# kscalelabs/kbot-joystick

Hardware: NVIDIA B200
Metric: env-steps/sec (obs + LSTM actor/critic + torque + terminations + rewards + GAE) (higher is better)
Workload: dtype f32 (tcgen05 2xFP16-split GEMMs, fp32 accumulate)

## Files before the change

### kbot-joystick_b200/csrc/kbs_net_tc.cu

```cuda
#include <math.h>
#include <cuda.h>
#include <stdlib.h>

#include "kbs_common.cuh"

namespace {

constexpr int kPanelRows = 128;
constexpr int kTileCols = 128;
constexpr int kUnitsPerTile = 32;
#ifndef KBS_STAGES
#define KBS_STAGES 6
#endif
constexpr int kStages = KBS_STAGES;
constexpr int kABlockBytes = 2 * 4 * kPanelRows * 16;
constexpr int kBBlockBytes = 2 * 4 * kTileCols * 16;
constexpr int kStageBytes = kABlockBytes + kBBlockBytes;
static_assert(kABlockBytes == kBBlockBytes, "the two producer lanes copy equal-sized blocks");
constexpr int kIssuers = 3;
constexpr int kProducers = 2;
constexpr int kEpiWarps = 8;
constexpr int kThreadsTC = 32 * (kIssuers + kProducers + kEpiWarps);
constexpr int kMaxBias = 1024;
constexpr int kSmemBytes = kStages * kStageBytes + 2 * kMaxBias * 4 + 256  + 1024 ;
// ... 566 lines not shown
      float m = out_s[lane * 41 + j] + P.joint_bias[j];
      m = m + in_arm[jj];
      const float y = in_lpf[jj];
      const float yn = y + P.lpf_alpha * (m - y);
      a.lpf[o] = rst ? 0.0f : yn;
      float act = yn;
      if (a.eps) act = yn + sd * in_eps[jj];
      const float a_eval = a.action_in ? in_ain[jj] : act;
      const float z = (a_eval - yn) / sd;
      s_z = s_z + (-0.5f * z * z - kHalfLog2Pi);
      s_log = s_log + logf(sd);
      if (a.action) a.action[o] = act;
      if (a.std) a.std[o] = sd;
      if (!a.ctrl) continue;
      const float target = a.ep.action_bias ? __fadd_rn(act, in_ab[jj]) : act;
      float tau = __fsub_rn(__fmul_rn(in_kp[jj], __fsub_rn(target, in_q[jj])), __fmul_rn(in_kd[jj], in_qd[jj]));
      if (a.ep.torque_bias) tau = __fadd_rn(tau, in_tb[jj]);
      a.ctrl[o] = fminf(fmaxf(tau, -in_lim[jj]), in_lim[jj]);
    }
  }
  part[(g * 32 + lane) * 2] = s_z;
  part[(g * 32 + lane) * 2 + 1] = s_log;
  __syncthreads();
  if (g == 0 && live) {
    float z = 0.0f, l = 0.0f;
#pragma unroll
    for (int w = 0; w < 4; ++w) { z = z + part[(w * 32 + lane) * 2]; l = l + part[(w * 32 + lane) * 2 + 1]; }
    if (a.log_prob) a.log_prob[e] = z - l;
    if (a.entropy) a.entropy[e] = l + float(KBS_NUM_JOINTS) * (0.5f + kHalfLog2Pi);
  }
}

constexpr int kPMaxDepth = 2;
constexpr int kPBiasFloats = 2 * kPMaxDepth * kMaxBias + 2 * 256;
constexpr int kEpiWarpsP = 16;
constexpr int kIssuersP = 1;
constexpr int kProducersP = 1;
constexpr int kThreadsP = 32 * (kIssuersP + kProducersP + kEpiWarpsP + 2);
constexpr int kPHeadPartFloats = 4 * kPanelRows * 2;
constexpr int kTileColsP = 256;
constexpr int kUnitsPerTileP = kTileColsP / 4;
constexpr int kBBlockBytesP = 2 * 4 * kTileColsP * 16;
constexpr int kStageBytesP = kABlockBytes + kBBlockBytesP;
constexpr int kStagesP = 4;
constexpr int kPSmemBytes = kStagesP * kStageBytesP + (kPBiasFloats + kPHeadPartFloats) * 4 + 256  + 1024 ;

struct PNet {
  const char* x_sb_all;
  size_t x0_stride;
  int kb_x0;
  char* hsb;
  char* xmid;
  float* fb;
  const char* w_sb[kPMaxDepth];
  const float* bias_t[kPMaxDepth];
  const char* w_head;
  const float* bias_head;
  unsigned int* flags;
  float* c_hist;
  float* save_g;
};
struct PArgs {
  PNet net[2];
  int nets, depth, H, panels, tiles;
  int gpanels;
  int64_t n, ld, T;
  size_t sbb;
  const uint8_t* done;
  const float* arm_cmd;
  float* lpf;
  const float* eps;
  const float* q; const float* qd;
  kbs_episode_view ep;
  float* action; float* log_prob; float* ctrl; float* value;
  const float* action_in; float* entropy; float* std;
  float* mean;
  float* sraw;
  int hist;
  int dbg;
  unsigned int* status;
  long long* trace;
};

struct PItem { int kind, net, layer, panel, tile; int t; bool valid; };
__device__ __forceinline__ PItem p_decode(const PArgs& a, int g) {
  const int lt = a.depth * a.tiles, per_panel = lt + 1, per_net = a.gpanels * per_panel, C = a.nets * per_net;
  const int per_group = (int(a.T) + a.depth) * C;
  const int grp = g / per_group;
  g -= grp * per_group;
  const int s = g / C;
// ... 29 lines not shown
      tg[nd++] = (t - 1) * (l + 1 == a.depth ? full_h : full_l);
    }
  } else {
    fp[nd] = N.flags + (a.depth - 1) * a.panels + it.panel; tg[nd++] = (t + 1) * full_l;
    if (t >= 1) { fp[nd] = N.flags + a.depth * a.panels + it.panel; tg[nd++] = t * full_h; }
  }
  if (nd == 0) return 0;
  for (int i = nd; i < 3; ++i) { fp[i] = fp[0]; tg[i] = 0u; }
  const long long c0 = clock64();
  unsigned int polls = 0;
  unsigned long long t0 = 0;
  while (true) {
    const unsigned int v0 = ld_volatile_u32(fp[0]), v1 = ld_volatile_u32(fp[1]), v2 = ld_volatile_u32(fp[2]);
    if (v0 >= tg[0] && v1 >= tg[1] && v2 >= tg[2]) break;
    if ((++polls & 1023u) == 0u) {
      if (ld_volatile_u32(a.status) & 3u) { drain = true; break; }
      unsigned long long now;
      asm volatile("mov.u64 %0, %%globaltimer;" : "=l"(now));
      if (t0 == 0) t0 = now;
      else if (now - t0 > kPWaitTimeoutNs) { atomicOr(a.status, 1u + unsigned(it.kind)); drain = true; break; }
    }
  }
  __threadfence();
  return clock64() - c0;
}

template <int KIND, bool SAVE>
__global__ void __launch_bounds__(kThreadsP, 1)
rollout_persist_kernel(const __grid_constant__ kbs_params P, const __grid_constant__ PArgs args) {
  extern __shared__ uint8_t smem_raw[];
  uint8_t* smem = reinterpret_cast<uint8_t*>((reinterpret_cast<uintptr_t>(smem_raw) + 1023) & ~uintptr_t(1023));
  float* bias_s = reinterpret_cast<float*>(smem + kStagesP * kStageBytesP);
  float* bias_head_s = bias_s + 2 * kPMaxDepth * kMaxBias;
  float* head_part = bias_s + kPBiasFloats;
  uint64_t* bars = reinterpret_cast<uint64_t*>(smem + kStagesP * kStageBytesP + (kPBiasFloats + kPHeadPartFloats) * 4);
  uint64_t* full = bars;
  uint64_t* empty = bars + kStagesP;
  uint64_t* acc_full = bars + 2 * kStagesP;
  uint64_t* acc_empty = acc_full + 2;
  uint64_t* corr_init = acc_empty + 2;
  uint32_t* tmem_slot = reinterpret_cast<uint32_t*>(corr_init + 2);
  volatile int* dep_seq = reinterpret_cast<volatile int*>(tmem_slot + 1);
  unsigned int* epi_done = reinterpret_cast<unsigned int*>(tmem_slot + 2);

  const int warp = threadIdx.x >> 5, lane = threadIdx.x & 31;
  const int per_slot = args.nets * args.gpanels * (args.depth * args.tiles + 1);
  const int n_g = ((args.panels + args.gpanels - 1) / args.gpanels) * (int(args.T) + args.depth) * per_slot;
  const int H = args.H;
  constexpr int kBlk = kbs_block_k(KIND);
  const int kb = H / kBlk;
  long long* tr = args.trace ? args.trace + size_t(blockIdx.x) * 16 : nullptr;
  const long long t_start = clock64();
  unsigned long long gt_start = 0;
  if (tr && threadIdx.x == 0) asm volatile("mov.u64 %0, %%globaltimer;" : "=l"(gt_start));

  if (threadIdx.x == 0) {
    for (int s = 0; s < kStagesP; ++s) { mbar_init(&full[s], 1); mbar_init(&empty[s], 1); }
    for (int b = 0; b < 2; ++b) {
      mbar_init(&acc_full[b], 1); mbar_init(&acc_empty[b], kEpiWarpsP);
    }
    *dep_seq = 0;
    *epi_done = 0u;
    asm volatile("fence.mbarrier_init.release.cluster;" ::: "memory");
  }
  if (warp == 0) {
    asm volatile("tcgen05.alloc.cta_group::1.sync.aligned.shared::cta.b32 [%0], %1;" ::"r"(smem_u32(tmem_slot)),
// ... 14 lines not shown
        ++j;
        const unsigned int want = unsigned(j) * kEpiWarpsP;
        unsigned int seen;
        do {
          asm volatile("ld.acquire.cta.shared::cta.u32 %0, [%1];" : "=r"(seen) : "r"(smem_u32(epi_done)) : "memory");
        } while (seen < want);
        __threadfence();
        atomicAdd(args.net[it.net].flags + it.layer * args.panels + it.panel, unsigned(kEpiWarpsP));
      }
    }
    __syncwarp();
  } else if (warp == kIssuersP + kProducersP + kEpiWarpsP) {
    if (lane == 0) {
      int j = 0;
      long long waited = 0;
      bool drain = false;
      for (int gi = blockIdx.x; gi < n_g; gi += gridDim.x) {
        const PItem it = p_decode(args, gi);
        if (!it.valid) continue;
        if (!(args.dbg & 1)) waited += p_wait_deps(args, it, drain);
        *dep_seq = ++j;
      }
      if (tr) { tr[1] = waited; tr[2] = j; }
    }
    __syncwarp();
  } else if (warp >= kIssuersP && warp < kIssuersP + kProducersP) {
    if (lane < 2) {
      uint32_t g = 0;
      int j = 0;
      long long pw[3] = {0, 0, 0};
      for (int gi = blockIdx.x; gi < n_g; gi += gridDim.x) {
        const PItem it = p_decode(args, gi);
        if (!it.valid) continue;
        const PNet& N = args.net[it.net];
        const int kb_x = (it.kind == 0 && it.layer == 0) ? N.kb_x0 : kb;
        const int kb_total = it.kind == 0 ? kb_x + kb : kb;
        size_t poff = size_t(it.panel) * kb * kABlockBytes;
        if (args.dbg & 8) poff = size_t(blockIdx.x % args.panels) * kb * kABlockBytes;
        const char* xa; const char* ha; const char* wb;
        if (it.kind == 0) {
          const size_t xs = SAVE ? size_t(it.layer - 1) * size_t(args.T) + size_t(it.t) : size_t((it.layer - 1) * 2 + (it.t & 1));
          const size_t hs = SAVE ? size_t(it.layer) * size_t(args.T + 1) + size_t(it.t) : size_t(it.layer * 2 + (it.t & 1));
          xa = it.layer == 0 ? N.x_sb_all + size_t(it.t) * N.x0_stride + poff / kb * kb_x : N.xmid + xs * args.sbb + poff;
          ha = N.hsb + hs * args.sbb + poff;
          wb = N.w_sb[it.layer] + size_t((args.dbg & 16) ? (blockIdx.x + it.t) % args.tiles : it.tile) * kb_total * kBBlockBytesP;
        } else {
          xa = N.xmid + (SAVE ? size_t(args.depth - 1) * size_t(args.T) + size_t(it.t) : size_t((args.depth - 1) * 2 + (it.t & 1))) * args.sbb + poff;
          ha = xa;
          wb = N.w_head;
        }
        ++j;
        bool need_dep = true;
        for (int b = 0; b < kb_total; ++b, ++g) {
          const int s = g % kStagesP;
          const uint32_t wbytes = (args.dbg & 128) ? 0u : (args.dbg & 32) ? 16u : uint32_t(kBBlockBytesP);
          const uint32_t abytes = (args.dbg & 256) ? uint32_t(kABlockBytes / 2) : uint32_t(kABlockBytes);
          long long p0 = 0, p1 = 0;
          if (lane == 0) {
            if (tr) p0 = clock64();
            mbar_wait(&empty[s], ((g / kStagesP) & 1) ^ 1);
            if (tr) p1 = clock64();
            mbar_expect_tx(&full[s], abytes + wbytes);
          }
          __syncwarp(0x3);
          uint8_t* sa = smem + size_t(s) * kStageBytesP;
          const char* src = lane == 0 ? ((b < kb_x) ? xa + size_t(b) * kABlockBytes : ha + size_t(b - kb_x) * kABlockBytes)
                                      : wb + size_t(b) * kBBlockBytesP;
          if (lane == 0 && need_dep) {
            const long long d0 = tr ? clock64() : 0;
            while (*dep_seq < j) { }
            __threadfence_block();
            asm volatile("fence.proxy.async;" ::: "memory");
            if (tr) pw[2] += clock64() - d0;
            need_dep = false;
          }
          if (lane == 0 || wbytes) bulk_g2s(sa + lane * kABlockBytes, src, lane == 0 ? abytes : wbytes, &full[s]);
          if (tr && lane == 0) { pw[0] += p1 - p0; pw[1] += clock64() - p1; }
        }
      }
      if (tr && lane == 0 && warp == kIssuersP) { tr[12] = pw[0]; tr[13] = pw[1]; tr[14] = pw[2]; }
    }
    __syncwarp();
  } else if (warp < kIssuersP) {
    int j = 0;
    uint32_t ph = 0;
    long long waited = 0, waited_acc = 0;
    {
      const uint32_t smem_base = smem_u32(smem);
      const uint64_t a_hi = umma_desc(smem_base, 2048, 128);
      const uint64_t a_lo = a_hi + (8192 >> 4);
      const uint64_t b_hi = umma_desc(smem_base + kABlockBytes, 8192, 128);
      const uint64_t b_lo = b_hi + (4096 >> 4);
      constexpr uint64_t kStageDesc = uint64_t(kStageBytesP) >> 4;
      constexpr uint64_t kAStep = 4096 >> 4, kBStep = 16384 >> 4;
      for (int gi = blockIdx.x; gi < n_g; gi += gridDim.x) {
        const PItem it = p_decode(args, gi);
        if (!it.valid) continue;
        const int kb_total = it.kind == 0 ? ((it.layer == 0 ? args.net[it.net].kb_x0 : kb) + kb) : kb;
        const long long e0 = tr ? clock64() : 0;
        mbar_wait(&acc_empty[0], (j & 1) ^ 1);
        if (tr) waited_acc += clock64() - e0;
        tc_fence_after();
        const uint32_t d_main = tmem_base, d_corr = tmem_base + kTileColsP;
        for (int b0 = 0; b0 < kb_total; b0 += kStagesP) {
#pragma unroll
          for (int st = 0; st < kStagesP; ++st) {
            const long long w0 = tr ? clock64() : 0;
            mbar_wait(&full[st], ph);
            if (tr) waited += clock64() - w0;
            tc_fence_after();
            const uint64_t so = st * kStageDesc;
            if (elect_one()) {
              if (!(args.dbg & 64)) {
                const uint32_t acc = (b0 | st) != 0;
                umma<KIND, kTileColsP>(d_main, a_hi + so, b_hi + so, acc);
                umma<KIND, kTileColsP>(d_corr, a_lo + so, b_hi + so, acc);
                umma<KIND, kTileColsP>(d_corr, a_hi + so, b_lo + so, 1);
                umma<KIND, kTileColsP>(d_main, a_hi + so + kAStep, b_hi + so + kBStep, 1);
                umma<KIND, kTileColsP>(d_corr, a_lo + so + kAStep, b_hi + so + kBStep, 1);
                umma<KIND, kTileColsP>(d_corr, a_hi + so + kAStep, b_lo + so + kBStep, 1);
              }
              umma_commit(&empty[st]);
            }
            __syncwarp();
          }
          ph ^= 1;
        }
        if (elect_one()) umma_commit(&acc_full[0]);
        __syncwarp();
        ++j;
      }
      if (tr && lane == 0) { tr[3] = waited; tr[7] = waited_acc; }
    }
  } else {
    const int ew = warp - kIssuersP - kProducersP;
    {
      const int et = threadIdx.x - 32 * (kIssuersP + kProducersP);
      for (int k = 0; k < args.nets; ++k) {
        for (int l = 0; l < args.depth; ++l)
          for (int i = et * 4; i < 4 * H; i += 32 * kEpiWarpsP * 4)
            *reinterpret_cast<float4*>(bias_s + (k * kPMaxDepth + l) * kMaxBias + i) =
                *reinterpret_cast<const float4*>(args.net[k].bias_t[l] + i);
        if (et < kTileColsP) bias_head_s[k * kTileColsP + et] = args.net[k].bias_head[et];
      }
      asm volatile("bar.sync 1, %0;" ::"n"(32 * kEpiWarpsP) : "memory");
    }
    const int q4 = warp & 3, grp = ew >> 2;
    const int r = q4 * 32 + lane;
    constexpr float kCorr = (KIND == KBS_KIND_F16) ? (1.0f / kKbsF16LoScale) : 1.0f;
    const int64_t ld = args.ld;
    const int colq = grp * 64;
    int j = 0;
    long long epi_cyc[2] = {0, 0}, epi_wait = 0, ph[4] = {0, 0, 0, 0};
    for (int gi = blockIdx.x; gi < n_g; gi += gridDim.x) {
      const PItem it = p_decode(args, gi);
      if (!it.valid) continue;
      const PNet& N = args.net[it.net];
      const int64_t R = int64_t(it.panel) * kPanelRows + r;
      const bool live = R < args.n;
      const int u0 = it.tile * kUnitsPerTileP + grp * 16;
      while (*dep_seq < j + 1) { }
      __threadfence_block();
      const size_t npH = size_t(args.panels) * kPanelRows * H;
      float* cst = SAVE ? N.c_hist + (size_t(it.layer) * size_t(args.T + 1) + size_t(it.kind == 0 ? it.t : 0)) * npH
                        : N.fb + size_t(it.layer) * 2 * npH;
      float* cdst = SAVE ? cst + npH : cst;
      float4 cpre[4];
      if (it.kind == 0 && live) {
#pragma unroll
        for (int q = 0; q < 4; ++q) cpre[q] = __ldcg(reinterpret_cast<const float4*>(cst + fb_offset(R, u0 + q * 4, H)));
      }
      const uint8_t* done_t = args.done ? args.done + size_t(it.t) * ld : nullptr;
      const bool rst = live && done_t && done_t[R];
      bool published = false;
      const long long ew0 = tr ? clock64() : 0;
      mbar_wait(&acc_full[0], j & 1);
      const long long ew1 = tr ? clock64() : 0;
      tc_fence_after();
      const uint32_t tq = tmem_base + (uint32_t(q4 * 32) << 16) + uint32_t(colq);
      if (it.kind == 0) {
        float v[64];
#pragma unroll
        for (int g4 = 0; g4 < 4; ++g4) {
          float cr[16];
          tmem_ld16(tq + 16 * g4, v + 16 * g4);
          tmem_ld16(tq + kTileColsP + 16 * g4, cr);
          tmem_ld_wait();
#pragma unroll
          for (int i = 0; i < 16; ++i) v[16 * g4 + i] += kCorr * cr[i];
        }
        tc_fence_before();
        __syncwarp();
        if (lane == 0) mbar_arrive(&acc_empty[0]);
        if (tr) ph[0] += clock64() - ew1;
        const float* bs = bias_s + (it.net * kPMaxDepth + it.layer) * kMaxBias + it.tile * kTileColsP + colq;
#pragma unroll
        for (int i = 0; i < 64; ++i) v[i] += bs[i];
        if (live && !(args.dbg & 2)) {
          char* x_out = N.xmid + (SAVE ? size_t(it.layer) * size_t(args.T) + size_t(it.t) : size_t(it.layer * 2 + (it.t & 1))) * args.sbb;
          char* h_out = N.hsb + (SAVE ? size_t(it.layer) * size_t(args.T + 1) + size_t(it.t + 1)
                                      : size_t(it.layer * 2 + ((it.t + 1) & 1))) * args.sbb;
          float* h_carry = (!SAVE && it.t == int(args.T) - 1) ? cst + npH : nullptr;
#pragma unroll
          for (int hf = 0; hf < 2; ++hf) {
            float hn[8], cn[8];
            if (SAVE) {
              float ai[8], af[8], ag[8], ao[8];
#pragma unroll
              for (int i = 0; i < 8; ++i) {
                const int u = hf * 8 + i;
                const float cprev = (&cpre[u >> 2].x)[u & 3];
                ai[i] = sigmoidf_(v[u]); af[i] = sigmoidf_(v[16 + u]); ag[i] = tanhf_(v[32 + u]); ao[i] = sigmoidf_(v[48 + u]);
                cn[i] = af[i] * cprev + ai[i] * ag[i];
                hn[i] = ao[i] * tanhf_(cn[i]);
                if (rst) cn[i] = 0.0f;
              }
#pragma unroll
              for (int i = 0; i < 8; ++i) {
                const int u = hf * 8 + i;
                v[u] = ai[i]; v[16 + u] = af[i]; v[32 + u] = ag[i]; v[48 + u] = ao[i];
              }
            } else {
#pragma unroll
            for (int i = 0; i < 8; ++i) {
              const int u = hf * 8 + i;
              const float cprev = (&cpre[u >> 2].x)[u & 3];
              const float gi_ = v[u], gf = v[16 + u], gg = v[32 + u], go = v[48 + u];
              cn[i] = sigmoidf_(gf) * cprev + sig_mul_tanh(gi_, gg);
              hn[i] = sig_mul_tanh(go, cn[i]);
              if (rst) cn[i] = 0.0f;
            }
            }
            if (!((args.dbg & 4) && hn[0] != 12345.0f)) {
              const int uu = u0 + hf * 8;
              const float h0[4] = {hn[0], hn[1], hn[2], hn[3]}, h1[4] = {hn[4], hn[5], hn[6], hn[7]};
              const KbsSplit4 s0 = sb_split4<KIND>(h0), s1 = sb_split4<KIND>(h1);
              sb_store_split8<kPanelRows, KIND>(x_out, R, uu, kb, s0, s1, false);
              sb_store_split8<kPanelRows, KIND>(h_out, R, uu, kb, s0, s1, rst);
              *reinterpret_cast<float4*>(cdst + fb_offset(R, uu, H)) = make_float4(cn[0], cn[1], cn[2], cn[3]);
              *reinterpret_cast<float4*>(cdst + fb_offset(R, uu + 4, H)) = make_float4(cn[4], cn[5], cn[6], cn[7]);
              if (h_carry) {
                const float z = rst ? 0.0f : 1.0f;
                *reinterpret_cast<float4*>(h_carry + fb_offset(R, uu, H)) = make_float4(z * hn[0], z * hn[1], z * hn[2], z * hn[3]);
                *reinterpret_cast<float4*>(h_carry + fb_offset(R, uu + 4, H)) = make_float4(z * hn[4], z * hn[5], z * hn[6], z * hn[7]);
              }
            }
          }
        }
        if (SAVE) {
          __syncwarp();
          if (lane == 0) asm volatile("red.release.cta.shared::cta.add.u32 [%0], 1;" ::"r"(smem_u32(epi_done)) : "memory");
          published = true;
          if (live && !(args.dbg & 2)) {
            float* sg = N.save_g + (size_t(it.t) * args.depth + it.layer) * 4 * npH;
#pragma unroll
            for (int gate = 0; gate < 4; ++gate)
#pragma unroll
              for (int q = 0; q < 4; ++q)
                *reinterpret_cast<float4*>(sg + gate * npH + fb_offset(R, u0 + 4 * q, H)) =
                    make_float4(v[16 * gate + 4 * q], v[16 * gate + 4 * q + 1], v[16 * gate + 4 * q + 2], v[16 * gate + 4 * q + 3]);
          }
        }
      } else {
        float v[16];
        {
          float cr[16];
          tmem_ld8(tq, v); tmem_ld8(tq + 16, v + 8);
          tmem_ld8(tq + kTileColsP, cr); tmem_ld8(tq + kTileColsP + 16, cr + 8);
          tmem_ld_wait();
#pragma unroll
          for (int i = 0; i < 16; ++i) v[i] += kCorr * cr[i];
        }
        tc_fence_before();
        __syncwarp();
        if (lane == 0) mbar_arrive(&acc_empty[0]);
        const float* bs = bias_head_s + it.net * kTileColsP + colq;
        const int64_t e = R;
        const size_t t = size_t(it.t);
        float s_z = 0.0f, s_log = 0.0f;
        if (it.net == 1) {
          if (live && grp == 0) args.value[t * ld + e] = v[0] + bs[0];
        } else {
          constexpr float kHalfLog2Pi = 0.918938533204672742f;
          if (live) {
            const int j0 = 5 * grp;
            float in_lpf[5], in_eps[5], in_arm[5], in_ain[5], in_q[5], in_qd[5], in_kp[5], in_kd[5], in_lim[5], in_ab[5], in_tb[5];
#pragma unroll
            for (int jj = 0; jj < 5; ++jj) {
              const int jn = j0 + jj;
              const int64_t o = jn * ld + e;
              in_lpf[jj] = __ldcg(args.lpf + o);
              in_eps[jj] = args.eps ? __ldg(args.eps + t * KBS_NUM_JOINTS * ld + o) : 0.0f;
              in_arm[jj] = (jn >= 10) ? __ldg(args.arm_cmd + t * KBS_ACTOR_OBS * ld + (jn - 10) * ld + e) : 0.0f;
              in_ain[jj] = args.action_in ? __ldg(args.action_in + t * KBS_NUM_JOINTS * ld + o) : 0.0f;
              if (args.ctrl) {
                in_q[jj] = __ldg(args.q + t * KBS_NQ * ld + o);
                in_qd[jj] = __ldg(args.qd + t * KBS_NV * ld + o);
                in_kp[jj] = args.ep.kp ? __ldg(args.ep.kp + o) : P.kp[jn];
                in_kd[jj] = args.ep.kd ? __ldg(args.ep.kd + o) : P.kd[jn];
                in_lim[jj] = args.ep.tau_limit ? __ldg(args.ep.tau_limit + o) : P.ctrl_limit[jn];
                in_ab[jj] = args.ep.action_bias ? __ldg(args.ep.action_bias + o) : 0.0f;
                in_tb[jj] = args.ep.torque_bias ? __ldg(args.ep.torque_bias + o) : 0.0f;
              }
            }
#pragma unroll
            for (int jj = 0; jj < 5; ++jj) {
              const int jn = j0 + jj;
              const int64_t o = jn * ld + e;
// ... 15 lines not shown
              if (args.std) args.std[t * KBS_NUM_JOINTS * ld + o] = sd;
              if (args.mean) args.mean[t * KBS_NUM_JOINTS * ld + o] = yn;
              if (SAVE && args.sraw) args.sraw[t * KBS_NUM_JOINTS * ld + o] = sraw;
              if (args.ctrl) {
                const float target = args.ep.action_bias ? __fadd_rn(act, in_ab[jj]) : act;
                float tau = __fsub_rn(__fmul_rn(in_kp[jj], __fsub_rn(target, in_q[jj])), __fmul_rn(in_kd[jj], in_qd[jj]));
                if (args.ep.torque_bias) tau = __fadd_rn(tau, in_tb[jj]);
                args.ctrl[t * KBS_NUM_JOINTS * ld + o] = fminf(fmaxf(tau, -in_lim[jj]), in_lim[jj]);
              }
            }
          }
          head_part[(grp * kPanelRows + r) * 2] = s_z;
          head_part[(grp * kPanelRows + r) * 2 + 1] = s_log;
          asm volatile("bar.sync %0, 128;" ::"r"(2 + q4) : "memory");
          if (grp == 0 && live) {
            float z = 0.0f, l = 0.0f;
#pragma unroll
            for (int w = 0; w < 4; ++w) { z = z + head_part[(w * kPanelRows + r) * 2]; l = l + head_part[(w * kPanelRows + r) * 2 + 1]; }
            if (args.log_prob) args.log_prob[t * ld + e] = z - l;
            if (args.entropy) args.entropy[t * ld + e] = l + float(KBS_NUM_JOINTS) * (0.5f + kHalfLog2Pi);
          }
          asm volatile("bar.sync %0, 128;" ::"r"(2 + q4) : "memory");
        }
      }
      const long long ew2 = tr ? clock64() : 0;
      __syncwarp();
      long long ewf = 0;
      if (lane == 0 && !published) {
        asm volatile("red.release.cta.shared::cta.add.u32 [%0], 1;" ::"r"(smem_u32(epi_done)) : "memory");
        if (tr) ewf = clock64();
      }
      if (tr) { const long long ew3 = clock64(); epi_cyc[it.kind] += ew3 - ew1; epi_wait += ew1 - ew0; if (it.kind == 0) { ph[1] += ew2 - ew1; ph[2] += ew3 - ew2; ph[3] += ewf - ew2; } }
      ++j;
    }
    if (tr && threadIdx.x == 32 * (kIssuersP + kProducersP)) { tr[4] = epi_cyc[0]; tr[5] = epi_cyc[1]; tr[6] = epi_wait; tr[8] = ph[0]; tr[9] = ph[1]; tr[10] = ph[2]; tr[11] = ph[3]; }
  }
  tc_fence_before();
  __syncthreads();
  if (tr && threadIdx.x == 0) {
    unsigned long long gt_end;
    asm volatile("mov.u64 %0, %%globaltimer;" : "=l"(gt_end));
    tr[0] = clock64() - t_start;
    tr[15] = (long long)(gt_end - gt_start);
  }
  if (warp == 0) {
    asm volatile("tcgen05.dealloc.cta_group::1.sync.aligned.b32 %0, %1;" ::"r"(tmem_base), "r"(512u));
  }
}

constexpr int kBT = 64;
template <int BT> struct BTile {
  static constexpr int kBBlockBytes = 2 * 4 * BT * 16;
  static constexpr int kStageBytes = kABlockBytes + kBBlockBytes;
  static constexpr int kStages = BT == 64 ? 8 : 6;
  static constexpr int kSmemBytes = kStages * kStageBytes + 256  + 1024 ;
};
constexpr int kBEpiWarps = 16;
constexpr int kBThreads = 32 * (1 + 1 + kBEpiWarps + 2);
struct BNet {
  const char* w_bwd[kPMaxDepth];
  char* dG;
  const float* save_g;
  const float* c_hist;
  const float* dh_top;
  const float* dv;
  const float* w_out;
// ... 1043 lines not shown
  sb_store4<TILE, KIND, true>(w_sb, col, k, Kp / kbs_block_k(KIND), x);
  if (k == 0) bias_t[col] = col < H ? b[col] : 0.0f;
}

struct FPackLayout {
  int kb;
  int fbase[kFMaxBlocks];
  short nvalid[kFMaxBlocks];
};
template <int KIND>
__global__ void __launch_bounds__(256)
pack_proj_weights_kmap_kernel(const float* __restrict__ w, int ldw, const float* __restrict__ b, const __grid_constant__ FPackLayout L,
                              char* __restrict__ w_sb, float* __restrict__ bias_t, int H, int Kq) {
  constexpr int kf = kbs_block_k(KIND);
  const int kq = Kq / 4;
  const int64_t idx = int64_t(blockIdx.x) * 256 + threadIdx.x;
  if (idx >= int64_t(256) * kq) return;
  const int col = int(idx / kq), k = int(idx % kq) * 4;
  float x[4] = {0.f, 0.f, 0.f, 0.f};
  if (col < H) {
#pragma unroll
    for (int i = 0; i < 4; ++i) {
      const int blk = (k + i) / kf, j = (k + i) % kf;
      x[i] = j < L.nvalid[blk] ? w[size_t(col) * ldw + L.fbase[blk] + j] : 0.0f;
    }
  }
  sb_store4<256, KIND, true>(w_sb, col, k, Kq / kf, x);
  if (k == 0) bias_t[col] = col < H ? b[col] : 0.0f;
}

template <int KIND>
__global__ void __launch_bounds__(256)
pack_head_weights_kernel(const float* __restrict__ w, const float* __restrict__ b, char* __restrict__ w_sb,
                         float* __restrict__ bias_t, int H, int num_out) {
  const int kq = H / 4;
  const int64_t idx = int64_t(blockIdx.x) * 256 + threadIdx.x;
  if (idx >= int64_t(kTileColsP) * kq) return;
  const int col = int(idx / kq), k = int(idx % kq) * 4;
  const int grp = col / 64, gate = (col % 64) / 16, uu = col % 16;
  int row = -1;
  if (gate < 2 && uu < 5) row = gate * KBS_NUM_JOINTS + grp * 5 + uu;
  if (row >= num_out) row = -1;
  float x[4] = {0.f, 0.f, 0.f, 0.f};
  if (row >= 0) {
#pragma unroll
    for (int i = 0; i < 4; ++i) x[i] = w[size_t(row) * H + k + i];
  }
  sb_store4<kTileColsP, KIND, true>(w_sb, col, k, H / kbs_block_k(KIND), x);
  if (k == 0) bias_t[col] = row >= 0 ? b[row] : 0.0f;
}

__global__ void __launch_bounds__(256)
fb_convert_kernel(float* __restrict__ rm, float* __restrict__ fb, int64_t n, int64_t n_pad, int H, int to_fb) {
  const int hq = H / 4;
  const int64_t idx = int64_t(blockIdx.x) * 256 + threadIdx.x;
  if (idx >= n_pad * hq) return;
  const int64_t panel = idx / (int64_t(kPanelRows) * hq);
  const int rem = int(idx - panel * int64_t(kPanelRows) * hq);
  const int kc = rem / kPanelRows, r = rem % kPanelRows;
  const int64_t row = panel * kPanelRows + r;
  float4* f = reinterpret_cast<float4*>(fb + fb_offset(row, kc * 4, H));
  if (to_fb) {
    *f = row < n ? *reinterpret_cast<const float4*>(rm + row * H + kc * 4) : make_float4(0.f, 0.f, 0.f, 0.f);
  } else if (row < n) {
    *reinterpret_cast<float4*>(rm + row * H + kc * 4) = *f;
  }
}

template <int KIND>
__global__ void __launch_bounds__(256)
pack_rows_sb_kernel(const float* __restrict__ src, int64_t ld, char* __restrict__ sb, int64_t n, int64_t n_pad, int K) {
  const int kq = K / 4;
  const int64_t idx = int64_t(blockIdx.x) * 256 + threadIdx.x;
  if (idx >= n_pad * kq) return;
  const int64_t panel = idx / (int64_t(kPanelRows) * kq);
  const int rem = int(idx - panel * int64_t(kPanelRows) * kq);
  const int kc = rem / kPanelRows, r = rem % kPanelRows;
  const int64_t row = panel * kPanelRows + r;
  float x[4] = {0.f, 0.f, 0.f, 0.f};
  if (row < n) {
    const float4 v = *reinterpret_cast<const float4*>(src + row * ld + kc * 4);
    x[0] = v.x; x[1] = v.y; x[2] = v.z; x[3] = v.w;
// ... 295 lines not shown
}

static inline int tc_kind(const kbs_handle* h) { return h->p.gemm_path == KBS_GEMM_TC_2XF16 ? KBS_KIND_F16 : KBS_KIND_TF32; }
static inline int proj_kp(const kbs_handle* h, int net) {
  return round_up_i(h->net[net].num_in, kbs_block_k(tc_kind(h)));
}
static size_t layer_image_bytes(const kbs_handle* h) {
  const int H = h->p.hidden_size;
  return kbs_sb_bytes_kind(tc_kind(h), 4 * H, 2 * H) + size_t(4 * H) * 4;
}
static inline int proj_cols(const kbs_handle* h) { return round_up_i(h->p.hidden_size, kTileCols); }
static size_t proj_image_bytes(const kbs_handle* h, int net) {
  return kbs_sb_bytes_kind(tc_kind(h), proj_cols(h), proj_kp(h, net)) + size_t(proj_cols(h)) * 4;
}
static inline char* layer_w(const kbs_handle* h, int net, int l) {
  return reinterpret_cast<char*>(h->net[net].tc_image) + layer_image_bytes(h) * l;
}
static inline float* layer_bias(const kbs_handle* h, int net, int l) {
  const int H = h->p.hidden_size;
  return reinterpret_cast<float*>(layer_w(h, net, l) + kbs_sb_bytes_kind(tc_kind(h), 4 * H, 2 * H));
}
static inline char* proj_w(const kbs_handle* h, int net) { return layer_w(h, net, h->p.depth); }
static inline float* proj_bias(const kbs_handle* h, int net) {
  return reinterpret_cast<float*>(proj_w(h, net) + kbs_sb_bytes_kind(tc_kind(h), proj_cols(h), proj_kp(h, net)));
}
static inline char* layer_w_p(const kbs_handle* h, int net, int l) {
  return proj_w(h, net) + proj_image_bytes(h, net) + layer_image_bytes(h) * l;
}
static inline float* layer_bias_p(const kbs_handle* h, int net, int l) {
  const int H = h->p.hidden_size;
  return reinterpret_cast<float*>(layer_w_p(h, net, l) + kbs_sb_bytes_kind(tc_kind(h), 4 * H, 2 * H));
}
static size_t head_image_bytes(const kbs_handle* h) {
  return kbs_sb_bytes_kind(tc_kind(h), kTileColsP, h->p.hidden_size) + size_t(kTileColsP) * 4;
}
static inline char* head_w(const kbs_handle* h, int net) { return layer_w_p(h, net, h->p.depth); }
static inline float* head_bias(const kbs_handle* h, int net) {
  return reinterpret_cast<float*>(head_w(h, net) + kbs_sb_bytes_kind(tc_kind(h), kTileColsP, h->p.hidden_size));
}
static inline int fused_kp(const kbs_handle* h, int net) { return round_up_i(h->net[net].num_in, 4 * kbs_block_k(tc_kind(h))); }
static inline bool fused_shape(const kbs_handle* h, int net) { return fused_kp(h, net) < h->p.hidden_size; }
static size_t fused_image_bytes(const kbs_handle* h, int net) {
  if (!fused_shape(h, net)) return 0;
  const int H = h->p.hidden_size, Kf = fused_kp(h, net);
  return size_t(4 * H) * Kf * 4 + size_t(4 * H) * 4 + kbs_sb_bytes_kind(tc_kind(h), 4 * H, Kf + H) + size_t(4 * H) * 4;
}
static inline float* fused_wf(const kbs_handle* h, int net) {
  return reinterpret_cast<float*>(head_w(h, net) + head_image_bytes(h));
}
static inline float* fused_bf(const kbs_handle* h, int net) { return fused_wf(h, net) + size_t(4 * h->p.hidden_size) * fused_kp(h, net); }
static inline char* fused_w(const kbs_handle* h, int net) { return reinterpret_cast<char*>(fused_bf(h, net) + 4 * h->p.hidden_size); }
static inline float* fused_bias(const kbs_handle* h, int net) {
  return reinterpret_cast<float*>(fused_w(h, net) + kbs_sb_bytes_kind(tc_kind(h), 4 * h->p.hidden_size, fused_kp(h, net) + h->p.hidden_size));
}
struct FLayout {
  int kb = 0;
  signed char src[kFMaxBlocks];
  short row0[kFMaxBlocks], nvalid[kFMaxBlocks];
  int fbase[kFMaxBlocks];
};
static inline bool projq_shape(const kbs_handle* h) { return h->p.hidden_size == 256; }
static FLayout projq_layout(const kbs_handle* h, int net, int which) {
  FLayout L;
  const int kf = kbs_block_k(tc_kind(h)), F = h->net[net].num_in;
  auto region = [&](int src, int start, int count, int f_base) {
    for (int i = 0; i * kf < count; ++i) {
      const int b = L.kb++;
      L.src[b] = (signed char)src; L.row0[b] = short(start + i * kf);
      L.nvalid[b] = short(count - i * kf < kf ? count - i * kf : kf);
      L.fbase[b] = f_base + i * kf;
    }
  };
// ... 114 lines not shown
      const int Kq = projq_kq(h, net, which);
      FPackLayout P{};
      P.kb = L.kb;
      for (int b = 0; b < L.kb; ++b) { P.fbase[b] = L.fbase[b]; P.nvalid[b] = L.nvalid[b]; }
      const int64_t total = int64_t(256) * (Kq / 4);
      const unsigned gb = unsigned((total + 255) / 256);
      if (kind == KBS_KIND_TF32)
        KBS_LAUNCH(h, KBS_K_PACK, st, (pack_proj_weights_kmap_kernel<KBS_KIND_TF32><<<gb, 256, 0, st>>>(
                                          N.w_in, N.kin_pad, N.b_in, P, projq_w(h, net, which), projq_bias(h, net, which), H, Kq)));
      else
        KBS_LAUNCH(h, KBS_K_PACK, st, (pack_proj_weights_kmap_kernel<KBS_KIND_F16><<<gb, 256, 0, st>>>(
                                          N.w_in, N.kin_pad, N.b_in, P, projq_w(h, net, which), projq_bias(h, net, which), H, Kq)));
    }
  }
  if (persist_shape_ok(h) && fused_shape(h, net)) {
    const int Kf = fused_kp(h, net);
    const int64_t tot_f = int64_t(4 * H) * (Kf + 1);
    KBS_LAUNCH(h, KBS_K_PACK, st, (fuse_input_weights_kernel<<<unsigned((tot_f + 255) / 256), 256, 0, st>>>(
                                      N.w_ih[0], N.w_in, N.kin_pad, N.num_in, N.b_in, N.b[0], fused_wf(h, net), fused_bf(h, net), H, Kf)));
    const int64_t total = int64_t(4 * H) * ((Kf + H) / 4);
    const unsigned gb = unsigned((total + 255) / 256);
    if (kind == KBS_KIND_TF32)
      KBS_LAUNCH(h, KBS_K_PACK, st, (pack_lstm_weights_kernel<KBS_KIND_TF32, kTileColsP><<<gb, 256, 0, st>>>(
                                        fused_wf(h, net), N.w_hh[0], fused_bf(h, net), fused_w(h, net), fused_bias(h, net), H, Kf, Kf)));
    else
      KBS_LAUNCH(h, KBS_K_PACK, st, (pack_lstm_weights_kernel<KBS_KIND_F16, kTileColsP><<<gb, 256, 0, st>>>(
                                        fused_wf(h, net), N.w_hh[0], fused_bf(h, net), fused_w(h, net), fused_bias(h, net), H, Kf, Kf)));
  }
  if (persist_shape_ok(h)) {
    const int64_t total = int64_t(kTileColsP) * (H / 4);
    const unsigned gb = unsigned((total + 255) / 256);
    if (kind == KBS_KIND_TF32)
      KBS_LAUNCH(h, KBS_K_PACK, st, (pack_head_weights_kernel<KBS_KIND_TF32><<<gb, 256, 0, st>>>(
                                        N.w_out, N.b_out, head_w(h, net), head_bias(h, net), H, N.num_out)));
    else
      KBS_LAUNCH(h, KBS_K_PACK, st, (pack_head_weights_kernel<KBS_KIND_F16><<<gb, 256, 0, st>>>(
                                        N.w_out, N.b_out, head_w(h, net), head_bias(h, net), H, N.num_out)));
  }
  KBS_LAUNCH_CHECK();
  return KBS_OK;
}

static int pack_rows(kbs_handle* h, const float* src, int64_t ld, char* sb, int64_t n, int64_t np, int K, cudaStream_t st) {
  const int64_t chunks = np * (K / 4);
  const unsigned gb = unsigned((chunks + 255) / 256);
  if (tc_kind(h) == KBS_KIND_TF32)
    KBS_LAUNCH(h, KBS_K_PACK, st, (pack_rows_sb_kernel<KBS_KIND_TF32><<<gb, 256, 0, st>>>(src, ld, sb, n, np, K)));
  else
    KBS_LAUNCH(h, KBS_K_PACK, st, (pack_rows_sb_kernel<KBS_KIND_F16><<<gb, 256, 0, st>>>(src, ld, sb, n, np, K)));
  return KBS_OK;
}

static size_t act_sb_bytes(const kbs_handle* h, int64_t n) { return kbs_sb_bytes_kind(tc_kind(h), pad_rows(n), h->p.hidden_size); }

size_t kbs_tc_scratch_floats(const kbs_handle* h, int64_t n) {
  const size_t H = size_t(h->p.hidden_size);
  return act_sb_bytes(h, n) / 4 * (2 + 2 * size_t(h->p.depth)) + 2 * size_t(h->p.depth) * size_t(pad_rows(n)) * H +
         2 * size_t(n) * H + 256;
}

static int fb_convert(kbs_handle* h, float* rm, float* fb, int64_t n, int64_t np, int H, int to_fb, cudaStream_t st) {
  const int64_t tot = np * (H / 4);
  KBS_LAUNCH(h, KBS_K_PACK, st, (fb_convert_kernel<<<unsigned((tot + 255) / 256), 256, 0, st>>>(rm, fb, n, np, H, to_fb)));
  return KBS_OK;
}

static int carry_convert(kbs_handle* h, const CarryJobs& J, int jobs, int64_t n, int64_t np, int H, cudaStream_t st) {
  const int kt = (H / 8 + 31) / 32;
  const dim3 grid(unsigned((np / 32) * kt), unsigned(jobs));
  if (tc_kind(h) == KBS_KIND_TF32)
// ... 830 lines not shown
      for (int l = 0; l < depth; ++l) {
        char* h_dst = hsb[k] + sbb * (hstep * l);
        float* c_dst = r.save ? r.c_hist[k] + fbf * (hstep * l) : fb[k] + fbf * (2 * l);
        if (!r.carry[k]) {
          KBS_CUDA_TRY(cudaMemsetAsync(h_dst, 0, sbb, st));
          KBS_CUDA_TRY(cudaMemsetAsync(c_dst, 0, fbf * sizeof(float), st));
          continue;
        }
        J.rm[j] = r.carry[k] + (size_t(l) * 2 + 0) * slot_f; J.blk[j] = h_dst; J.mode[j++] = 0;
        J.rm[j] = r.carry[k] + (size_t(l) * 2 + 1) * slot_f; J.blk[j] = c_dst; J.mode[j++] = 1;
      }
    if (j) carry_convert(h, J, j, n, np, H, st);
  } else {
    for (int k = 0; k < nets; ++k)
      for (int l = 0; l < depth; ++l) {
        pack_rows(h, r.carry[k] + (size_t(l) * 2 + 0) * size_t(n) * H, H, hsb[k] + sbb * (2 * l), n, np, H, st);
        fb_convert(h, r.carry[k] + (size_t(l) * 2 + 1) * size_t(n) * H, fb[k] + fbf * (2 * l), n, np, H, 1, st);
      }
  }
  const int panels = int(np / kPanelRows), tiles = H / kUnitsPerTileP;
  if (persistent) {
    if (r.chunk_len > 0)
      for (int64_t c = 0; c * r.chunk_len < r.T; ++c) KBS_CUDA_TRY(cudaStreamWaitEvent(st, r.chunk_events[c], 0));
    PArgs a{};
    for (int k = 0; k < nets; ++k) {
      PNet& N = a.net[k];
      N.x_sb_all = reinterpret_cast<const char*>(r.x_sb_all[k]);
      N.kb_x0 = r.x_is_obs[k] ? fused_kp(h, k) / kbs_block_k(kind) : H / kbs_block_k(kind);
      N.x0_stride = r.x_is_obs[k] ? kbs_sb_bytes_kind(kind, np, fused_kp(h, k)) : sbb;
      N.hsb = hsb[k]; N.xmid = xmid[k]; N.fb = fb[k]; N.flags = flags[k];
      N.c_hist = r.save ? r.c_hist[k] : nullptr; N.save_g = r.save ? r.save_g[k] : nullptr;
      for (int l = 0; l < depth; ++l) { N.w_sb[l] = layer_w_p(h, k, l); N.bias_t[l] = layer_bias_p(h, k, l); }
      if (r.x_is_obs[k]) { N.w_sb[0] = fused_w(h, k); N.bias_t[0] = fused_bias(h, k); }
      N.w_head = head_w(h, k); N.bias_head = head_bias(h, k);
      KBS_CUDA_TRY(cudaMemsetAsync(flags[k], 0, rollout_flag_bytes(h, n), st));
    }
    a.nets = nets; a.depth = depth; a.H = H; a.panels = panels; a.tiles = tiles;
    a.n = n; a.ld = ld; a.T = r.T; a.sbb = sbb;
    {
      int gp = panels;
      const char* e = getenv("KBS_PERSIST_GROUP");
      if (e) { const int v = atoi(e); gp = (v <= 0 || v > panels) ? panels : v; }
      a.gpanels = gp;
    }
    a.done = r.done;
    a.arm_cmd = r.actor_obs + size_t(55) * ld;
    a.lpf = r.lpf; a.eps = r.eps_action;
    a.q = r.qpos ? r.qpos + size_t(7) * ld : nullptr;
    a.qd = r.qvel ? r.qvel + size_t(6) * ld : nullptr;
    a.ep = r.ep;
    a.action = r.action; a.log_prob = r.log_prob; a.ctrl = (r.ctrl && r.qpos && r.qvel) ? r.ctrl : nullptr; a.value = r.value;
    a.action_in = r.action_in; a.entropy = r.entropy; a.std = r.action_std; a.mean = r.mean;
    a.sraw = r.save ? r.sraw : nullptr; a.hist = r.save ? 1 : 0;
    a.status = h->persist_status;
    { const char* e = getenv("KBS_PERSIST_DBG"); a.dbg = e ? atoi(e) : 0; }
    a.trace = h->trace_buf;
    cudaLaunchConfig_t cfg{};
    const int64_t per_slot = int64_t(nets) * a.gpanels * (depth * tiles + 1);
    cfg.gridDim = dim3(unsigned(per_slot < h->num_sms ? per_slot : h->num_sms));
    { const char* e = getenv("KBS_PERSIST_GRID"); if (e && atoi(e) > 0 && atoi(e) < int(cfg.gridDim.x)) cfg.gridDim.x = unsigned(atoi(e)); }
    cfg.blockDim = dim3(kThreadsP);
    cfg.dynamicSmemBytes = kPSmemBytes;
    cfg.stream = st;
    cudaLaunchAttribute at[1];
    at[0].id = cudaLaunchAttributeCooperative;
    at[0].val.cooperative = 1;
    cfg.attrs = at;
// ... 123 lines not shown
```

Measured before the change: 68.46 million.

## Fold critic value head into last LSTM layer epilogue in non-save rollout

In the persistent rollout kernel without SAVE, the critic's scalar value head is computed as a dot product inside the last LSTM layer's epilogue instead of a separate tensor-core head GEMM. Each tile writes a per-tile partial sum to a scratch buffer that reuses the last layer's xmid storage. The head item then just sums the partials, so it skips the producer copies, the MMA and the TMEM round-trip, and the last layer no longer stores its split activations to xmid. In exchange the epilogue gains an extra FMA loop and two named barriers per panel, and the head result now depends on partial sums staying correctly ordered across tiles.

```diff
diff --git a/kbot-joystick_b200/csrc/kbs_net_tc.cu b/kbot-joystick_b200/csrc/kbs_net_tc.cu
--- a/kbot-joystick_b200/csrc/kbs_net_tc.cu
+++ b/kbot-joystick_b200/csrc/kbs_net_tc.cu
@@ -622,7 +622,7 @@
 }
 
 constexpr int kPMaxDepth = 2;
-constexpr int kPBiasFloats = 2 * kPMaxDepth * kMaxBias + 2 * 256;
+constexpr int kPBiasFloats = 2 * kPMaxDepth * kMaxBias + 2 * 256 + 256;
 constexpr int kEpiWarpsP = 16;
 constexpr int kIssuersP = 1;
 constexpr int kProducersP = 1;
@@ -646,6 +646,8 @@
   const float* bias_t[kPMaxDepth];
   const char* w_head;
   const float* bias_head;
+  const float* w_head_f;
+  float* hpart;
   unsigned int* flags;
   float* c_hist;
   float* save_g;
@@ -741,6 +743,7 @@
   uint8_t* smem = reinterpret_cast<uint8_t*>((reinterpret_cast<uintptr_t>(smem_raw) + 1023) & ~uintptr_t(1023));
   float* bias_s = reinterpret_cast<float*>(smem + kStagesP * kStageBytesP);
   float* bias_head_s = bias_s + 2 * kPMaxDepth * kMaxBias;
+  float* w_crit_s = bias_head_s + 2 * kTileColsP;
   float* head_part = bias_s + kPBiasFloats;
   uint64_t* bars = reinterpret_cast<uint64_t*>(smem + kStagesP * kStageBytesP + (kPBiasFloats + kPHeadPartFloats) * 4);
   uint64_t* full = bars;
@@ -821,6 +824,7 @@
       for (int gi = blockIdx.x; gi < n_g; gi += gridDim.x) {
         const PItem it = p_decode(args, gi);
         if (!it.valid) continue;
+        if (!SAVE && it.kind == 1 && it.net == 1) { ++j; continue; }
         const PNet& N = args.net[it.net];
         const int kb_x = (it.kind == 0 && it.layer == 0) ? N.kb_x0 : kb;
         const int kb_total = it.kind == 0 ? kb_x + kb : kb;
@@ -884,7 +888,7 @@
       constexpr uint64_t kAStep = 4096 >> 4, kBStep = 16384 >> 4;
       for (int gi = blockIdx.x; gi < n_g; gi += gridDim.x) {
         const PItem it = p_decode(args, gi);
-        if (!it.valid) continue;
+        if (!it.valid || (!SAVE && it.kind == 1 && it.net == 1)) continue;
         const int kb_total = it.kind == 0 ? ((it.layer == 0 ? args.net[it.net].kb_x0 : kb) + kb) : kb;
         const long long e0 = tr ? clock64() : 0;
         mbar_wait(&acc_empty[0], (j & 1) ^ 1);
@@ -932,6 +936,8 @@
                 *reinterpret_cast<const float4*>(args.net[k].bias_t[l] + i);
         if (et < kTileColsP) bias_head_s[k * kTileColsP + et] = args.net[k].bias_head[et];
       }
+      if (args.nets > 1)
+        for (int i = et; i < H; i += 32 * kEpiWarpsP) w_crit_s[i] = args.net[1].w_head_f[i];
       asm volatile("bar.sync 1, %0;" ::"n"(32 * kEpiWarpsP) : "memory");
     }
     const int q4 = warp & 3, grp = ew >> 2;
@@ -939,7 +945,7 @@
     constexpr float kCorr = (KIND == KBS_KIND_F16) ? (1.0f / kKbsF16LoScale) : 1.0f;
     const int64_t ld = args.ld;
     const int colq = grp * 64;
-    int j = 0;
+    int j = 0, ja = 0;
     long long epi_cyc[2] = {0, 0}, epi_wait = 0, ph[4] = {0, 0, 0, 0};
     for (int gi = blockIdx.x; gi < n_g; gi += gridDim.x) {
       const PItem it = p_decode(args, gi);
@@ -962,8 +968,10 @@
       const uint8_t* done_t = args.done ? args.done + size_t(it.t) * ld : nullptr;
       const bool rst = live && done_t && done_t[R];
       bool published = false;
+      const bool mma = SAVE || it.kind == 0 || it.net == 0;
+      const bool fold = !SAVE && it.kind == 0 && it.net == 1 && it.layer == args.depth - 1;
       const long long ew0 = tr ? clock64() : 0;
-      mbar_wait(&acc_full[0], j & 1);
+      if (mma) mbar_wait(&acc_full[0], ja & 1);
       const long long ew1 = tr ? clock64() : 0;
       tc_fence_after();
       const uint32_t tq = tmem_base + (uint32_t(q4 * 32) << 16) + uint32_t(colq);
@@ -985,6 +993,7 @@
         const float* bs = bias_s + (it.net * kPMaxDepth + it.layer) * kMaxBias + it.tile * kTileColsP + colq;
 #pragma unroll
         for (int i = 0; i < 64; ++i) v[i] += bs[i];
+        float crit = 0.0f;
         if (live && !(args.dbg & 2)) {
           char* x_out = N.xmid + (SAVE ? size_t(it.layer) * size_t(args.T) + size_t(it.t) : size_t(it.layer * 2 + (it.t & 1))) * args.sbb;
           char* h_out = N.hsb + (SAVE ? size_t(it.layer) * size_t(args.T + 1) + size_t(it.t + 1)
@@ -1020,11 +1029,15 @@
               if (rst) cn[i] = 0.0f;
             }
             }
+            if (fold) {
+#pragma unroll
+              for (int i = 0; i < 8; ++i) crit = fmaf(w_crit_s[u0 + hf * 8 + i], hn[i], crit);
+            }
             if (!((args.dbg & 4) && hn[0] != 12345.0f)) {
               const int uu = u0 + hf * 8;
               const float h0[4] = {hn[0], hn[1], hn[2], hn[3]}, h1[4] = {hn[4], hn[5], hn[6], hn[7]};
               const KbsSplit4 s0 = sb_split4<KIND>(h0), s1 = sb_split4<KIND>(h1);
-              sb_store_split8<kPanelRows, KIND>(x_out, R, uu, kb, s0, s1, false);
+              if (!fold) sb_store_split8<kPanelRows, KIND>(x_out, R, uu, kb, s0, s1, false);
               sb_store_split8<kPanelRows, KIND>(h_out, R, uu, kb, s0, s1, rst);
               *reinterpret_cast<float4*>(cdst + fb_offset(R, uu, H)) = make_float4(cn[0], cn[1], cn[2], cn[3]);
               *reinterpret_cast<float4*>(cdst + fb_offset(R, uu + 4, H)) = make_float4(cn[4], cn[5], cn[6], cn[7]);
@@ -1036,6 +1049,19 @@
             }
           }
         }
+        if (fold) {
+          float sum = crit;
+          if (grp != 0) head_part[(grp - 1) * kPanelRows + r] = sum;
+          asm volatile("bar.sync %0, 128;" ::"r"(2 + q4) : "memory");
+          if (grp == 0 && live) {
+            sum = sum + head_part[r];
+            sum = sum + head_part[kPanelRows + r];
+            sum = sum + head_part[2 * kPanelRows + r];
+            const size_t np = size_t(args.panels) * kPanelRows;
+            N.hpart[(size_t(it.tile) * 2 + size_t(it.t & 1)) * np + size_t(R)] = sum;
+          }
+          asm volatile("bar.sync %0, 128;" ::"r"(2 + q4) : "memory");
+        }
         if (SAVE) {
           __syncwarp();
           if (lane == 0) asm volatile("red.release.cta.shared::cta.add.u32 [%0], 1;" ::"r"(smem_u32(epi_done)) : "memory");
@@ -1052,17 +1078,23 @@
         }
       } else {
         float v[16];
-        {
+        if (mma) {
           float cr[16];
           tmem_ld8(tq, v); tmem_ld8(tq + 16, v + 8);
           tmem_ld8(tq + kTileColsP, cr); tmem_ld8(tq + kTileColsP + 16, cr + 8);
           tmem_ld_wait();
 #pragma unroll
           for (int i = 0; i < 16; ++i) v[i] += kCorr * cr[i];
-        }
-        tc_fence_before();
-        __syncwarp();
-        if (lane == 0) mbar_arrive(&acc_empty[0]);
+          tc_fence_before();
+          __syncwarp();
+          if (lane == 0) mbar_arrive(&acc_empty[0]);
+        } else if (live && grp == 0) {
+          const size_t np = size_t(args.panels) * kPanelRows;
+          const float* src = N.hpart + size_t(it.t & 1) * np + size_t(R);
+          float sum = __ldcg(src);
+          for (int tile = 1; tile < args.tiles; ++tile) sum = sum + __ldcg(src + size_t(tile) * 2 * np);
+          v[0] = sum;
+        }
         const float* bs = bias_head_s + it.net * kTileColsP + colq;
         const int64_t e = R;
         const size_t t = size_t(it.t);
@@ -1144,6 +1176,7 @@
       }
       if (tr) { const long long ew3 = clock64(); epi_cyc[it.kind] += ew3 - ew1; epi_wait += ew1 - ew0; if (it.kind == 0) { ph[1] += ew2 - ew1; ph[2] += ew3 - ew2; ph[3] += ewf - ew2; } }
       ++j;
+      if (mma) ++ja;
     }
     if (tr && threadIdx.x == 32 * (kIssuersP + kProducersP)) { tr[4] = epi_cyc[0]; tr[5] = epi_cyc[1]; tr[6] = epi_wait; tr[8] = ph[0]; tr[9] = ph[1]; tr[10] = ph[2]; tr[11] = ph[3]; }
   }
@@ -2253,7 +2286,7 @@
 template <int KIND>
 __global__ void __launch_bounds__(256)
 pack_head_weights_kernel(const float* __restrict__ w, const float* __restrict__ b, char* __restrict__ w_sb,
-                         float* __restrict__ bias_t, int H, int num_out) {
+                         float* __restrict__ bias_t, float* __restrict__ w_f, int H, int num_out) {
   const int kq = H / 4;
   const int64_t idx = int64_t(blockIdx.x) * 256 + threadIdx.x;
   if (idx >= int64_t(kTileColsP) * kq) return;
@@ -2269,6 +2302,10 @@
   }
   sb_store4<kTileColsP, KIND, true>(w_sb, col, k, H / kbs_block_k(KIND), x);
   if (k == 0) bias_t[col] = row >= 0 ? b[row] : 0.0f;
+  if (col == 0) {
+#pragma unroll
+    for (int i = 0; i < 4; ++i) w_f[k + i] = x[i];
+  }
 }
 
 __global__ void __launch_bounds__(256)
@@ -2630,12 +2667,13 @@
   return reinterpret_cast<float*>(layer_w_p(h, net, l) + kbs_sb_bytes_kind(tc_kind(h), 4 * H, 2 * H));
 }
 static size_t head_image_bytes(const kbs_handle* h) {
-  return kbs_sb_bytes_kind(tc_kind(h), kTileColsP, h->p.hidden_size) + size_t(kTileColsP) * 4;
+  return kbs_sb_bytes_kind(tc_kind(h), kTileColsP, h->p.hidden_size) + size_t(kTileColsP) * 4 + size_t(h->p.hidden_size) * 4;
 }
 static inline char* head_w(const kbs_handle* h, int net) { return layer_w_p(h, net, h->p.depth); }
 static inline float* head_bias(const kbs_handle* h, int net) {
   return reinterpret_cast<float*>(head_w(h, net) + kbs_sb_bytes_kind(tc_kind(h), kTileColsP, h->p.hidden_size));
 }
+static inline float* head_wf(const kbs_handle* h, int net) { return head_bias(h, net) + kTileColsP; }
 static inline int fused_kp(const kbs_handle* h, int net) { return round_up_i(h->net[net].num_in, 4 * kbs_block_k(tc_kind(h))); }
 static inline bool fused_shape(const kbs_handle* h, int net) { return fused_kp(h, net) < h->p.hidden_size; }
 static size_t fused_image_bytes(const kbs_handle* h, int net) {
@@ -2816,10 +2854,10 @@
     const unsigned gb = unsigned((total + 255) / 256);
     if (kind == KBS_KIND_TF32)
       KBS_LAUNCH(h, KBS_K_PACK, st, (pack_head_weights_kernel<KBS_KIND_TF32><<<gb, 256, 0, st>>>(
-                                        N.w_out, N.b_out, head_w(h, net), head_bias(h, net), H, N.num_out)));
+                                        N.w_out, N.b_out, head_w(h, net), head_bias(h, net), head_wf(h, net), H, N.num_out)));
     else
       KBS_LAUNCH(h, KBS_K_PACK, st, (pack_head_weights_kernel<KBS_KIND_F16><<<gb, 256, 0, st>>>(
-                                        N.w_out, N.b_out, head_w(h, net), head_bias(h, net), H, N.num_out)));
+                                        N.w_out, N.b_out, head_w(h, net), head_bias(h, net), head_wf(h, net), H, N.num_out)));
   }
   KBS_LAUNCH_CHECK();
   return KBS_OK;
@@ -3716,7 +3754,8 @@
       N.c_hist = r.save ? r.c_hist[k] : nullptr; N.save_g = r.save ? r.save_g[k] : nullptr;
       for (int l = 0; l < depth; ++l) { N.w_sb[l] = layer_w_p(h, k, l); N.bias_t[l] = layer_bias_p(h, k, l); }
       if (r.x_is_obs[k]) { N.w_sb[0] = fused_w(h, k); N.bias_t[0] = fused_bias(h, k); }
-      N.w_head = head_w(h, k); N.bias_head = head_bias(h, k);
+      N.w_head = head_w(h, k); N.bias_head = head_bias(h, k); N.w_head_f = head_wf(h, k);
+      N.hpart = r.save ? nullptr : reinterpret_cast<float*>(xmid[k] + sbb * 2 * (depth - 1));
       KBS_CUDA_TRY(cudaMemsetAsync(flags[k], 0, rollout_flag_bytes(h, n), st));
     }
     a.nets = nets; a.depth = depth; a.H = H; a.panels = panels; a.tiles = tiles;
```

Result: no change. 69.20 million, median of 6 (+1.1%).
